# Cuberick-Orion/Candidate-Reranking-CIR

Measured on NVIDIA B200. Metric: stage2_reranked_triplets_per_s, higher is better.
Workload: dtype bf16

## Files before the change

### candidate-reranking-cir_b200/csrc/rowops.cu

```cuda
#include "common.cuh"

namespace {

constexpr int D = CIR_HIDDEN;
constexpr int PER_LANE = D / 32;
constexpr int WARPS = 8;

template <typename T> __device__ __forceinline__ void load_row(const T* row, int lane, float (&v)[PER_LANE]);
template <> __device__ __forceinline__ void load_row<float>(const float* row, int lane, float (&v)[PER_LANE]) {
#pragma unroll
  for (int i = 0; i < 3; i++) {
    const float4* p = reinterpret_cast<const float4*>(row + (lane + 32 * i) * 8);
    const float4 a = p[0], b = p[1];
    v[8 * i] = a.x; v[8 * i + 1] = a.y; v[8 * i + 2] = a.z; v[8 * i + 3] = a.w;
    v[8 * i + 4] = b.x; v[8 * i + 5] = b.y; v[8 * i + 6] = b.z; v[8 * i + 7] = b.w;
  }
}
template <> __device__ __forceinline__ void load_row<bf16>(const bf16* row, int lane, float (&v)[PER_LANE]) {
  uint4 t[3];
#pragma unroll
  for (int i = 0; i < 3; i++) t[i] = *reinterpret_cast<const uint4*>(row + (lane + 32 * i) * 8);
#pragma unroll
  for (int i = 0; i < 3; i++) {
    const __nv_bfloat162* h = reinterpret_cast<const __nv_bfloat162*>(&t[i]);
#pragma unroll
    for (int q = 0; q < 4; q++) { float2 f = __bfloat1622float2(h[q]); v[8 * i + 2 * q] = f.x; v[8 * i + 2 * q + 1] = f.y; }
  }
}
template <typename T> __device__ __forceinline__ void store_row(T* row, int lane, const float (&v)[PER_LANE]);
template <> __device__ __forceinline__ void store_row<float>(float* row, int lane, const float (&v)[PER_LANE]) {
#pragma unroll
  for (int i = 0; i < 3; i++) {
    float4* p = reinterpret_cast<float4*>(row + (lane + 32 * i) * 8);
    p[0] = make_float4(v[8 * i], v[8 * i + 1], v[8 * i + 2], v[8 * i + 3]);
    p[1] = make_float4(v[8 * i + 4], v[8 * i + 5], v[8 * i + 6], v[8 * i + 7]);
  }
}
template <> __device__ __forceinline__ void store_row<bf16>(bf16* row, int lane, const float (&v)[PER_LANE]) {
#pragma unroll
  for (int i = 0; i < 3; i++) {
    uint4 t;
    __nv_bfloat162* h = reinterpret_cast<__nv_bfloat162*>(&t);
#pragma unroll
    for (int q = 0; q < 4; q++) h[q] = __floats2bfloat162_rn(v[8 * i + 2 * q], v[8 * i + 2 * q + 1]);
    *reinterpret_cast<uint4*>(row + (lane + 32 * i) * 8) = t;
  }
}

__device__ __forceinline__ void layernorm24(float (&v)[PER_LANE], const float* gamma, const float* beta, float eps, int lane) {
  float s = 0.f;
#pragma unroll
  for (int i = 0; i < PER_LANE; i++) s += v[i];
  const float mean = warp_sum(s) * (1.0f / D);
  float q = 0.f;
#pragma unroll
  for (int i = 0; i < PER_LANE; i++) { float d = v[i] - mean; q = fmaf(d, d, q); }
  const float rstd = rsqrtf(warp_sum(q) * (1.0f / D) + eps);
  float g[PER_LANE], b[PER_LANE];
  load_row<float>(gamma, lane, g);
  load_row<float>(beta, lane, b);
#pragma unroll
  for (int i = 0; i < PER_LANE; i++) v[i] = fmaf((v[i] - mean) * rstd, g[i], b[i]);
}

__device__ __forceinline__ uint64_t pk2(float lo, float hi) { uint64_t r; asm("mov.b64 %0, {%1, %2};" : "=l"(r) : "f"(lo), "f"(hi)); return r; }
__device__ __forceinline__ float lo2(uint64_t v) { float a, b; asm("mov.b64 {%0, %1}, %2;" : "=f"(a), "=f"(b) : "l"(v)); return a; }
__device__ __forceinline__ float hi2(uint64_t v) { float a, b; asm("mov.b64 {%0, %1}, %2;" : "=f"(a), "=f"(b) : "l"(v)); return b; }
__device__ __forceinline__ uint64_t add2(uint64_t a, uint64_t b) { uint64_t r; asm("add.rn.f32x2 %0, %1, %2;" : "=l"(r) : "l"(a), "l"(b)); return r; }
__device__ __forceinline__ uint64_t mul2(uint64_t a, uint64_t b) { uint64_t r; asm("mul.rn.f32x2 %0, %1, %2;" : "=l"(r) : "l"(a), "l"(b)); return r; }
__device__ __forceinline__ uint64_t fma2(uint64_t a, uint64_t b, uint64_t c) { uint64_t r; asm("fma.rn.f32x2 %0, %1, %2, %3;" : "=l"(r) : "l"(a), "l"(b), "l"(c)); return r; }

template <typename T> struct RawRow;
template <> struct RawRow<bf16> {
  uint4 q[3];
  __device__ __forceinline__ void load(const bf16* row, int lane) {
#pragma unroll
    for (int i = 0; i < 3; i++) q[i] = *reinterpret_cast<const uint4*>(row + (lane + 32 * i) * 8);
  }
  __device__ __forceinline__ void unpack(float (&v)[PER_LANE]) const {
#pragma unroll
    for (int i = 0; i < 3; i++) {
      const __nv_bfloat162* h = reinterpret_cast<const __nv_bfloat162*>(&q[i]);
#pragma unroll
      for (int k = 0; k < 4; k++) { float2 f = __bfloat1622float2(h[k]); v[8 * i + 2 * k] = f.x; v[8 * i + 2 * k + 1] = f.y; }
    }
  }
};
template <> struct RawRow<float> {
  float4 q[6];
  __device__ __forceinline__ void load(const float* row, int lane) {
#pragma unroll
    for (int i = 0; i < 3; i++) {
      const float4* p = reinterpret_cast<const float4*>(row + (lane + 32 * i) * 8);
      q[2 * i] = p[0]; q[2 * i + 1] = p[1];
    }
  }
  __device__ __forceinline__ void unpack(float (&v)[PER_LANE]) const {
#pragma unroll
    for (int i = 0; i < 6; i++) { v[4 * i] = q[i].x; v[4 * i + 1] = q[i].y; v[4 * i + 2] = q[i].z; v[4 * i + 3] = q[i].w; }
  }
};

constexpr int LN_ROWS = 4;
template <typename TX, typename TR, typename TY>
__global__ void __launch_bounds__(WARPS * 32)
add_layernorm_kernel(const TX* __restrict__ x, int64_t x_rows, const TR* __restrict__ res, const float* __restrict__ gamma,
                     const float* __restrict__ beta, int64_t rows_per_group, TY* __restrict__ y, int64_t rows, float eps) {
  const int lane = threadIdx.x & 31;
  const int64_t r0 = ((int64_t)blockIdx.x * WARPS + (threadIdx.x >> 5)) * LN_ROWS;
  if (r0 >= rows) return;
  const int n = (int)(rows - r0 < LN_ROWS ? rows - r0 : LN_ROWS);
  RawRow<TX> xr;
  RawRow<TR> rr;
  const uint32_t r32 = (uint32_t)r0;
  int64_t xi = (uint64_t)x_rows > (uint64_t)r0 ? r0 : (int64_t)(r32 % (uint32_t)x_rows);
  int64_t gr = (uint64_t)rows_per_group > (uint64_t)r0 ? 0 : (int64_t)(r32 / (uint32_t)rows_per_group);
  int64_t gleft = (gr + 1) * rows_per_group - r0;
  xr.load(x + xi * D, lane);
  if (res) rr.load(res + r0 * D, lane);
  float g[PER_LANE], b[PER_LANE];
  bool fresh = true;
#pragma unroll 1
  for (int i = 0; i < n; i++) {
    const int64_t r = r0 + i;
    float v[PER_LANE];
    xr.unpack(v);
    if (res) {
      float t[PER_LANE];
      rr.unpack(t);
#pragma unroll
      for (int k = 0; k < PER_LANE; k++) v[k] += t[k];
    }
    if (i + 1 < n) {
      xi = xi + 1 == x_rows ? 0 : xi + 1;
      xr.load(x + xi * D, lane);
      if (res) rr.load(res + (r + 1) * D, lane);
    }
    if (fresh) {
      fresh = false;
      load_row<float>(gamma + gr * D, lane, g);
      load_row<float>(beta + gr * D, lane, b);
    }
    if (--gleft == 0) { gr++; gleft = rows_per_group; fresh = true; }
    uint64_t v2[PER_LANE / 2];
#pragma unroll
    for (int k = 0; k < PER_LANE / 2; k++) v2[k] = pk2(v[2 * k], v[2 * k + 1]);
    uint64_t s2 = pk2(0.f, 0.f);
#pragma unroll
    for (int k = 0; k < PER_LANE / 2; k++) s2 = add2(s2, v2[k]);
    const float mean = warp_sum(lo2(s2) + hi2(s2)) * (1.0f / D);
    const uint64_t nmean2 = pk2(-mean, -mean);
    uint64_t q2 = pk2(0.f, 0.f);
#pragma unroll
    for (int k = 0; k < PER_LANE / 2; k++) { v2[k] = add2(v2[k], nmean2); q2 = fma2(v2[k], v2[k], q2); }
    const float rstd = rsqrtf(warp_sum(lo2(q2) + hi2(q2)) * (1.0f / D) + eps);
    const uint64_t rstd2 = pk2(rstd, rstd);
#pragma unroll
    for (int k = 0; k < PER_LANE / 2; k++) {
      const uint64_t o2 = fma2(mul2(v2[k], rstd2), pk2(g[2 * k], g[2 * k + 1]), pk2(b[2 * k], b[2 * k + 1]));
      v[2 * k] = lo2(o2); v[2 * k + 1] = hi2(o2);
    }
    store_row<TY>(y + r * D, lane, v);
  }
}

template <typename T>
__global__ void __launch_bounds__(WARPS * 32)
bert_embeddings_kernel(const int32_t* __restrict__ ids, int64_t rows, int64_t L, const float* __restrict__ word,
                       const float* __restrict__ pos, const float* __restrict__ gamma, const float* __restrict__ beta,
                       T* __restrict__ out) {
  const int lane = threadIdx.x & 31;
  const int64_t r = (int64_t)blockIdx.x * WARPS + (threadIdx.x >> 5);
  if (r >= rows) return;
  const int64_t l = r % L;
  float v[PER_LANE], t[PER_LANE];
  load_row<float>(word + (int64_t)ids[r] * D, lane, v);
  load_row<float>(pos + l * D, lane, t);
#pragma unroll
  for (int i = 0; i < PER_LANE; i++) v[i] += t[i];
  layernorm24(v, gamma, beta, 1e-12f, lane);
  store_row<T>(out + r * D, lane, v);
}

__global__ void gather_rows_kernel(const uint4* __restrict__ src, const int32_t* __restrict__ index, uint4* __restrict__ dst,
                                   int64_t rows, int64_t vecs) {
  const int64_t total = rows * vecs;
  for (int64_t i = (int64_t)blockIdx.x * blockDim.x + threadIdx.x; i < total; i += (int64_t)gridDim.x * blockDim.x) {
    const int64_t r = i / vecs, c = i - r * vecs;
    const int64_t s = index ? (int64_t)index[r] : r;
    dst[i] = src[s * vecs + c];
  }
}

template <typename TS, typename TD>
__global__ void cast_kernel(const TS* __restrict__ src, TD* __restrict__ dst, int64_t n) {
  for (int64_t i = (int64_t)blockIdx.x * blockDim.x + threadIdx.x; i < n; i += (int64_t)gridDim.x * blockDim.x)
    dst[i] = from_f32<TD>(to_f32<TS>(src[i]));
}

__global__ void l2_normalize_kernel(const float* __restrict__ x, float* __restrict__ y, int64_t rows, int64_t dim) {
  const int lane = threadIdx.x & 31;
  const int64_t r = (int64_t)blockIdx.x * WARPS + (threadIdx.x >> 5);
  if (r >= rows) return;
  float s = 0.f;
  for (int64_t i = lane; i < dim; i += 32) { float v = x[r * dim + i]; s = fmaf(v, v, s); }
  const float nrm = fmaxf(sqrtf(warp_sum(s)), 1e-12f);
  for (int64_t i = lane; i < dim; i += 32) y[r * dim + i] = x[r * dim + i] / nrm;
}

template <typename T>
__global__ void im2col16_kernel(const float* __restrict__ img, T* __restrict__ out, int64_t B, int S) {
  const int G = S / 16;
  const int64_t total = B * G * G * 192;
  for (int64_t i = (int64_t)blockIdx.x * blockDim.x + threadIdx.x; i < total; i += (int64_t)gridDim.x * blockDim.x) {
    const int v = (int)(i % 192);
    const int64_t pr = i / 192;
    const int px = (int)(pr % G), py = (int)((pr / G) % G);
    const int64_t b = pr / (G * G);
    const int c = v / 64, ky = (v % 64) / 4, kx = (v % 4) * 4;
    const float4 t = *reinterpret_cast<const float4*>(img + ((b * 3 + c) * S + (py * 16 + ky)) * (int64_t)S + px * 16 + kx);
    T* o = out + pr * 768 + c * 256 + ky * 16 + kx;
    o[0] = from_f32<T>(t.x); o[1] = from_f32<T>(t.y); o[2] = from_f32<T>(t.z); o[3] = from_f32<T>(t.w);
  }
}

__global__ void vit_assemble_kernel(const float* __restrict__ patch, const float* __restrict__ cls, const float* __restrict__ pos,
                                    float* __restrict__ x, int64_t B, int64_t N) {
  const int64_t total = B * N * (D / 4);
  for (int64_t i = (int64_t)blockIdx.x * blockDim.x + threadIdx.x; i < total; i += (int64_t)gridDim.x * blockDim.x) {
    const int c = (int)(i % (D / 4)) * 4;
    const int64_t r = i / (D / 4);
    const int64_t n = r % N, b = r / N;
    float4 a = (n == 0) ? *reinterpret_cast<const float4*>(cls + c)
                        : *reinterpret_cast<const float4*>(patch + (b * (N - 1) + n - 1) * D + c);
    const float4 p = *reinterpret_cast<const float4*>(pos + n * D + c);
    *reinterpret_cast<float4*>(x + r * D + c) = make_float4(a.x + p.x, a.y + p.y, a.z + p.z, a.w + p.w);
  }
}

template <typename T>
__global__ void gather_cls_kernel(const T* __restrict__ h, int64_t Tn, int64_t L, T* __restrict__ feats, float* __restrict__ feats_f32) {
  const int64_t total = Tn * 2 * D;
  for (int64_t i = (int64_t)blockIdx.x * blockDim.x + threadIdx.x; i < total; i += (int64_t)gridDim.x * blockDim.x) {
    const int c = (int)(i % D);
    const int s = (int)((i / D) % 2);
    const int64_t t = i / (2 * D);
    const T v = h[((int64_t)s * Tn * L + t * L) * D + c];
    feats[i] = v;
    if (feats_f32) feats_f32[i] = to_f32<T>(v);
  }
}

__global__ void __launch_bounds__(WARPS * 32)
head_dot_kernel(const float* __restrict__ hidden, const float* __restrict__ w, const float* __restrict__ b,
                float* __restrict__ scores, int64_t rows) {
  const int lane = threadIdx.x & 31;
  const int64_t r = (int64_t)blockIdx.x * WARPS + (threadIdx.x >> 5);
  if (r >= rows) return;
  float hv[PER_LANE], wv[PER_LANE];
  load_row<float>(hidden + r * D, lane, hv);
  load_row<float>(w, lane, wv);
  float s = 0.f;
#pragma unroll
  for (int i = 0; i < PER_LANE; i++) s = fmaf(hv[i], wv[i], s);
  s = warp_sum(s);
  if (lane == 0) scores[r] = s + b[0];
}

inline unsigned row_blocks(int64_t rows) { return (unsigned)((rows + WARPS - 1) / WARPS); }
inline unsigned flat_blocks(int64_t n, int threads = 256) {
  int64_t b = (n + threads - 1) / threads;
  return (unsigned)(b > 148 * 32 ? 148 * 32 : (b < 1 ? 1 : b));
}

}

extern "C" int cir_add_layernorm(cir_ctx* ctx, const void* x, int x_f32, int64_t x_rows, const void* res,
                                 const float* gamma, const float* beta, int64_t rows_per_group,
                                 void* y, int y_f32, int64_t rows, float eps) {
  CIR_ENTER(ctx);
  if (rows == 0) return CIR_OK;
  CIR_CHECK_ARG(x && gamma && beta && y && x_rows > 0 && rows_per_group > 0, "add_layernorm: null/zero argument");
  CIR_CHECK_ARG(rows < (1ll << 31), "add_layernorm: rows=%lld does not fit 32-bit row arithmetic", (long long)rows);
  const bool f32 = ctx->dtype == CIR_DTYPE_F32;
  dim3 grid(row_blocks((rows + LN_ROWS - 1) / LN_ROWS)), block(WARPS * 32);
  {
    const double es = f32 ? 4.0 : 2.0;
    cir_prof_begin(ctx, CIR_PROF_LAYERNORM, (double)rows * D * ((x_f32 ? 4.0 : es) + (res ? es : 0.0) + (y_f32 ? 4.0 : es)));
  }
#define LN_LAUNCH(TX, TR, TY) \
  add_layernorm_kernel<TX, TR, TY><<<grid, block, 0, ctx->stream>>>((const TX*)x, x_rows, (const TR*)res, gamma, beta, rows_per_group, (TY*)y, rows, eps)
  if (f32) LN_LAUNCH(float, float, float);
  else if (x_f32 && y_f32) LN_LAUNCH(float, bf16, float);
  else if (x_f32) LN_LAUNCH(float, bf16, bf16);
  else if (y_f32) LN_LAUNCH(bf16, bf16, float);
  else LN_LAUNCH(bf16, bf16, bf16);
#undef LN_LAUNCH
  cir_prof_end(ctx);
  CIR_LAUNCH_CHECK(ctx);
  return CIR_OK;
}

extern "C" int cir_bert_embeddings(cir_ctx* ctx, const int32_t* ids, int64_t Q, int64_t L, const float* word_emb,
                                   const float* pos_emb, const float* gamma, const float* beta, void* out) {
  CIR_ENTER(ctx);
  const int64_t rows = Q * L;
  if (rows == 0) return CIR_OK;
  CIR_CHECK_ARG(L <= 512, "bert_embeddings: L=%lld exceeds max_position_embeddings 512", (long long)L);
  if (ctx->dtype == CIR_DTYPE_F32)
    bert_embeddings_kernel<float><<<row_blocks(rows), WARPS * 32, 0, ctx->stream>>>(ids, rows, L, word_emb, pos_emb, gamma, beta, (float*)out);
  else
    bert_embeddings_kernel<bf16><<<row_blocks(rows), WARPS * 32, 0, ctx->stream>>>(ids, rows, L, word_emb, pos_emb, gamma, beta, (bf16*)out);
  CIR_LAUNCH_CHECK(ctx);
  return CIR_OK;
}

extern "C" int cir_gather_rows(cir_ctx* ctx, const void* src, const int32_t* index, void* dst, int64_t rows, int64_t row_elems) {
  CIR_ENTER(ctx);
  if (rows == 0 || row_elems == 0) return CIR_OK;
  const int64_t row_bytes = row_elems * (int64_t)act_size(ctx);
  CIR_CHECK_ARG(row_bytes % 16 == 0 && ((uintptr_t)src & 15) == 0 && ((uintptr_t)dst & 15) == 0, "gather_rows: rows must be 16 B multiples and aligned");
  const int64_t vecs = row_bytes / 16;
  gather_rows_kernel<<<flat_blocks(rows * vecs), 256, 0, ctx->stream>>>((const uint4*)src, index, (uint4*)dst, rows, vecs);
  CIR_LAUNCH_CHECK(ctx);
  return CIR_OK;
}

extern "C" int cir_cast_f32_to_act(cir_ctx* ctx, const float* src, void* dst, int64_t n) {
  CIR_ENTER(ctx);
  if (n == 0) return CIR_OK;
  if (ctx->dtype == CIR_DTYPE_F32) cast_kernel<float, float><<<flat_blocks(n), 256, 0, ctx->stream>>>(src, (float*)dst, n);
  else cast_kernel<float, bf16><<<flat_blocks(n), 256, 0, ctx->stream>>>(src, (bf16*)dst, n);
  CIR_LAUNCH_CHECK(ctx);
  return CIR_OK;
}

extern "C" int cir_cast_act_to_f32(cir_ctx* ctx, const void* src, float* dst, int64_t n) {
  CIR_ENTER(ctx);
  if (n == 0) return CIR_OK;
  if (ctx->dtype == CIR_DTYPE_F32) cast_kernel<float, float><<<flat_blocks(n), 256, 0, ctx->stream>>>((const float*)src, dst, n);
  else cast_kernel<bf16, float><<<flat_blocks(n), 256, 0, ctx->stream>>>((const bf16*)src, dst, n);
  CIR_LAUNCH_CHECK(ctx);
  return CIR_OK;
}

extern "C" int cir_l2_normalize(cir_ctx* ctx, const float* x, float* y, int64_t rows, int64_t dim) {
  CIR_ENTER(ctx);
  if (rows == 0) return CIR_OK;
  l2_normalize_kernel<<<row_blocks(rows), WARPS * 32, 0, ctx->stream>>>(x, y, rows, dim);
  CIR_LAUNCH_CHECK(ctx);
  return CIR_OK;
}

int cir_im2col16(cir_ctx* ctx, const float* img, void* out, int64_t B, int S) {
  const int64_t n = B * (S / 16) * (S / 16) * 192;
  if (ctx->dtype == CIR_DTYPE_F32) im2col16_kernel<float><<<flat_blocks(n), 256, 0, ctx->stream>>>(img, (float*)out, B, S);
  else im2col16_kernel<bf16><<<flat_blocks(n), 256, 0, ctx->stream>>>(img, (bf16*)out, B, S);
  CIR_LAUNCH_CHECK(ctx);
  return CIR_OK;
}
int cir_vit_assemble(cir_ctx* ctx, const float* patch, const float* cls, const float* pos, float* x, int64_t B, int64_t N) {
  vit_assemble_kernel<<<flat_blocks(B * N * (D / 4)), 256, 0, ctx->stream>>>(patch, cls, pos, x, B, N);
  CIR_LAUNCH_CHECK(ctx);
  return CIR_OK;
}
int cir_gather_cls(cir_ctx* ctx, const void* h, int64_t T, int64_t L, void* feats, float* feats_f32) {
  if (T == 0) return CIR_OK;
  if (ctx->dtype == CIR_DTYPE_F32) gather_cls_kernel<float><<<flat_blocks(T * 2 * D), 256, 0, ctx->stream>>>((const float*)h, T, L, (float*)feats, feats_f32);
  else gather_cls_kernel<bf16><<<flat_blocks(T * 2 * D), 256, 0, ctx->stream>>>((const bf16*)h, T, L, (bf16*)feats, feats_f32);
  CIR_LAUNCH_CHECK(ctx);
  return CIR_OK;
}
int cir_head_dot(cir_ctx* ctx, const float* hidden, const float* w, const float* b, float* scores, int64_t rows) {
  if (rows == 0) return CIR_OK;
  head_dot_kernel<<<row_blocks(rows), WARPS * 32, 0, ctx->stream>>>(hidden, w, b, scores, rows);
  CIR_LAUNCH_CHECK(ctx);
  return CIR_OK;
}
```

Before: 66090.

## Stage LayerNorm gamma/beta in shared memory, reverse block order, cap registers

The add+LayerNorm kernel now has each block cooperatively load the gamma/beta rows for the first and last group it covers into shared memory. Warps read these per row instead of keeping them in per-thread registers, with a fallback to global memory for any other group. Blocks are walked in reverse order, and launch bounds request three blocks per SM to cut register pressure. The trade-off is a __syncthreads, extra shared-memory traffic on every row, and possible spills under the tighter register budget.

```diff
diff --git a/candidate-reranking-cir_b200/csrc/rowops.cu b/candidate-reranking-cir_b200/csrc/rowops.cu
--- a/candidate-reranking-cir_b200/csrc/rowops.cu
+++ b/candidate-reranking-cir_b200/csrc/rowops.cu
@@ -103,11 +103,21 @@
 
 constexpr int LN_ROWS = 4;
 template <typename TX, typename TR, typename TY>
-__global__ void __launch_bounds__(WARPS * 32)
+__global__ void __launch_bounds__(WARPS * 32, 3)
 add_layernorm_kernel(const TX* __restrict__ x, int64_t x_rows, const TR* __restrict__ res, const float* __restrict__ gamma,
                      const float* __restrict__ beta, int64_t rows_per_group, TY* __restrict__ y, int64_t rows, float eps) {
   const int lane = threadIdx.x & 31;
-  const int64_t r0 = ((int64_t)blockIdx.x * WARPS + (threadIdx.x >> 5)) * LN_ROWS;
+  const int64_t blk_r0 = (int64_t)(gridDim.x - 1 - blockIdx.x) * WARPS * LN_ROWS;
+  const int64_t r0 = blk_r0 + (int64_t)(threadIdx.x >> 5) * LN_ROWS;
+  __shared__ __align__(16) float sgb[2][2][D];
+  const int64_t blk_r1 = (blk_r0 + WARPS * LN_ROWS < rows ? blk_r0 + WARPS * LN_ROWS : rows) - 1;
+  const int64_t g0 = (uint64_t)rows_per_group > (uint64_t)blk_r0 ? 0 : (int64_t)((uint32_t)blk_r0 / (uint32_t)rows_per_group);
+  const int64_t g1 = (uint64_t)rows_per_group > (uint64_t)blk_r1 ? 0 : (int64_t)((uint32_t)blk_r1 / (uint32_t)rows_per_group);
+  for (int c = threadIdx.x; c < D; c += WARPS * 32) {
+    sgb[0][0][c] = gamma[g0 * D + c]; sgb[0][1][c] = beta[g0 * D + c];
+    sgb[1][0][c] = gamma[g1 * D + c]; sgb[1][1][c] = beta[g1 * D + c];
+  }
+  __syncthreads();
   if (r0 >= rows) return;
   const int n = (int)(rows - r0 < LN_ROWS ? rows - r0 : LN_ROWS);
   RawRow<TX> xr;
@@ -118,8 +128,6 @@
   int64_t gleft = (gr + 1) * rows_per_group - r0;
   xr.load(x + xi * D, lane);
   if (res) rr.load(res + r0 * D, lane);
-  float g[PER_LANE], b[PER_LANE];
-  bool fresh = true;
 #pragma unroll 1
   for (int i = 0; i < n; i++) {
     const int64_t r = r0 + i;
@@ -136,12 +144,9 @@
       xr.load(x + xi * D, lane);
       if (res) rr.load(res + (r + 1) * D, lane);
     }
-    if (fresh) {
-      fresh = false;
-      load_row<float>(gamma + gr * D, lane, g);
-      load_row<float>(beta + gr * D, lane, b);
-    }
-    if (--gleft == 0) { gr++; gleft = rows_per_group; fresh = true; }
+    const float* gp = gr == g0 ? sgb[0][0] : gr == g1 ? sgb[1][0] : gamma + gr * D;
+    const float* bp = gr == g0 ? sgb[0][1] : gr == g1 ? sgb[1][1] : beta + gr * D;
+    if (--gleft == 0) { gr++; gleft = rows_per_group; }
     uint64_t v2[PER_LANE / 2];
 #pragma unroll
     for (int k = 0; k < PER_LANE / 2; k++) v2[k] = pk2(v[2 * k], v[2 * k + 1]);
@@ -156,9 +161,18 @@
     const float rstd = rsqrtf(warp_sum(lo2(q2) + hi2(q2)) * (1.0f / D) + eps);
     const uint64_t rstd2 = pk2(rstd, rstd);
 #pragma unroll
-    for (int k = 0; k < PER_LANE / 2; k++) {
-      const uint64_t o2 = fma2(mul2(v2[k], rstd2), pk2(g[2 * k], g[2 * k + 1]), pk2(b[2 * k], b[2 * k + 1]));
-      v[2 * k] = lo2(o2); v[2 * k + 1] = hi2(o2);
+    for (int i3 = 0; i3 < 3; i3++) {
+      const float4* g4 = reinterpret_cast<const float4*>(gp + (lane + 32 * i3) * 8);
+      const float4* b4 = reinterpret_cast<const float4*>(bp + (lane + 32 * i3) * 8);
+      const float4 ga = g4[0], gb = g4[1], ba = b4[0], bb = b4[1];
+      const float g[8] = {ga.x, ga.y, ga.z, ga.w, gb.x, gb.y, gb.z, gb.w};
+      const float b[8] = {ba.x, ba.y, ba.z, ba.w, bb.x, bb.y, bb.z, bb.w};
+#pragma unroll
+      for (int q = 0; q < 4; q++) {
+        const int k = 4 * i3 + q;
+        const uint64_t o2 = fma2(mul2(v2[k], rstd2), pk2(g[2 * q], g[2 * q + 1]), pk2(b[2 * q], b[2 * q + 1]));
+        v[2 * k] = lo2(o2); v[2 * k + 1] = hi2(o2);
+      }
     }
     store_row<TY>(y + r * D, lane, v);
   }
```

New measurement: 64450 (median of 6 runs). 0.975x the previous value.
